# tetriscode/cause

Measured on AMD Instinct MI355X. Metric: nodes woven/sec (whole node) + % of HBM roofline at 1/2/4/8 MI355X, higher is better.
Workload: dtype u64; 1 GPU; config2: independent CausalLists, full reweave; docs_per_gpu=10000, nodes_per_doc=50001, nodes_per_gpu=500010000, sites=8, key_bits=20, key_words=u64 (cw_weave_lists), parallelism=docs sharded x1

## Files before the change

### cause_amd/csrc/causeweave.hip

```cpp

#include <hip/hip_runtime.h>

#include <algorithm>
#include <type_traits>
#include <cstdarg>
#include <cstdio>
#include <cstdlib>
#include <cstring>
#include <map>
#include <chrono>
#include <string>
#include <vector>

#include "causeweave.h"
#include "cw_internal.h"

using namespace cw;


template <int NT>
__device__ __forceinline__ uint32_t block_exscan(uint32_t v, uint32_t *wtot, uint32_t *total) {
  const int nw = NT ? NT / 64 : (int)(blockDim.x >> 6);
  const uint32_t lane = threadIdx.x & 63, w = threadIdx.x >> 6;
  uint32_t x = v;
// ... 1066 lines not shown
  }
  if (tid == 0 && bst) atomicOr(&status[d], bst);
}

constexpr uint32_t KBM_WORDS = 2 * TILE / 32;
constexpr uint32_t FRONT_FUSED_SG = 2560;

template <int NT>
__global__ __launch_bounds__(NT) void k_fplace(
    const uint32_t *__restrict__ rec_meta, const uint32_t *__restrict__ rec_par,
    const uint32_t *__restrict__ woff, const uint32_t *__restrict__ woff_base,
    const uint32_t *__restrict__ tile_start, const uint32_t *__restrict__ tile_doc,
    const uint32_t *__restrict__ tile_first, const uint32_t *__restrict__ doc_off,
    const uint64_t *__restrict__ id_key, uint32_t *__restrict__ sval, uint32_t *__restrict__ par,
    uint8_t *__restrict__ skind, uint64_t *__restrict__ skey, uint32_t *__restrict__ kbm) {
  __shared__ uint32_t s_val[TILE], s_par[TILE];
  __shared__ uint8_t s_kind[TILE];
  __shared__ uint32_t s_run[65], s_src[64];
  const uint32_t t = xcd_tile(blockIdx.x, gridDim.x), d = tile_doc[t], tid = threadIdx.x;
  const uint32_t t0 = tile_first[d], ntile = tile_first[d + 1] - t0, w = t - t0;
  const uint32_t base = doc_off[d], n = doc_off[d + 1] - base;
  const uint32_t r0 = w << 12, wlen = min(TILE, n - r0);
  if (tid < 64) {
    uint32_t a = 0, l = 0;
    if (tid < ntile) {
      const uint32_t *wo = woff + woff_base[t0 + tid];
      a = wo[w];
      l = wo[w + 1] - a;
      s_src[tid] = tile_start[t0 + tid] + a;
    }
    uint32_t x = l;
#pragma unroll
    for (int o = 1; o < 64; o <<= 1) {
      const uint32_t y = __shfl_up(x, o, 64);
      if (tid >= (uint32_t)o) x += y;
    }
    s_run[tid + 1] = x;
    if (tid == 0) s_run[0] = 0;
  }
  for (uint32_t j = tid; j < wlen; j += NT) {
    s_val[j] = 0;
    s_par[j] = 0;
    s_kind[j] = 0;
  }
  __syncthreads();
  const uint32_t total = min(s_run[ntile], wlen);
  for (uint32_t j = tid; j < total; j += NT) {
    uint32_t lo = 0, hi = ntile;
    while (hi - lo > 1) {
      const uint32_t m = (lo + hi) >> 1;
      if (s_run[m] <= j) lo = m; else hi = m;
    }
    const uint32_t g = s_src[lo] + (j - s_run[lo]);
    const uint32_t meta = rec_meta[g], rr = meta & (TILE - 1);
    s_val[rr] = (lo << 12) | ((meta >> 12) & (TILE - 1));
    s_par[rr] = rec_par[g];
    s_kind[rr] = (uint8_t)(meta >> 24);
  }
  __syncthreads();
  for (uint32_t j = tid; j < wlen; j += NT) {
    const uint32_t v = s_val[j];
    sval[base + r0 + j] = v;
    par[base + r0 + j] = s_par[j];
    skind[base + r0 + j] = s_kind[j];
    if (skey) skey[base + r0 + j] = id_key[base + (v < n ? v : 0u)];
  }
  for (uint32_t j0 = (tid >> 6) << 6; j0 < TILE; j0 += NT) {
    const uint32_t j = j0 + (tid & 63);
    const uint8_t k = j < wlen ? s_kind[j] : 0;
    const uint64_t sm = __ballot(is_special(k)), hm = __ballot(is_hide(k));
    if ((tid & 63) == 0) {
      uint32_t *o = kbm + (size_t)t * KBM_WORDS + (j0 >> 5);
      o[0] = (uint32_t)sm;
      o[1] = (uint32_t)(sm >> 32);
      o[TILE / 32] = (uint32_t)hm;
      o[TILE / 32 + 1] = (uint32_t)(hm >> 32);
    }
  }
}

__host__ __device__ inline uint32_t front_lds_bytes(uint32_t nmax, uint32_t sg) {
  return sg * 16 + 4 * ((nmax + 1) / 2) + 8 * ((nmax + 31) / 32);
}

#ifndef CW_SITE8_RANKPASS
#define CW_SITE8_RANKPASS 0
#endif
constexpr bool SITE8_PASS1 = CW_SITE8_RANKPASS == 0;

template <int NT, typename PT = uint32_t, typename VT = uint32_t, uint32_t U1 = 4, uint32_t U2 = 4,
          uint32_t U3 = 4>
__device__ __forceinline__ bool front_doc(
    const uint64_t *__restrict__ id_key, const uint64_t *__restrict__ cause_key,
    const uint8_t *__restrict__ kind, const uint32_t *__restrict__ doc_off,
    const uint32_t *__restrict__ tile_first, uint32_t sg, PT *__restrict__ par,
    uint8_t *__restrict__ skind, VT *__restrict__ sval, uint32_t *__restrict__ kbm,
    uint64_t *__restrict__ skey, uint16_t *rank16, uint64_t *__restrict__ max_ts, uint32_t ts_shift,
    uint32_t *__restrict__ status, uint32_t *__restrict__ big,
    unsigned long long *__restrict__ tprof, uint32_t d, uint4 *sdir,
    uint8_t *__restrict__ site8 = nullptr, uint32_t site_shift = 0, uint32_t site_mask = 0) {
  unsigned long long tacc[6] = {0, 0, 0, 0, 0, 0}, tlast = 0;
  auto stamp = [&](int ph) {
    if (tprof) {
      const unsigned long long now = __builtin_amdgcn_s_memtime();
      if (ph >= 0) tacc[ph] += now - tlast;
      tlast = now;
    }
  };
  stamp(-1);
  __shared__ uint64_t rmax[NT / 64];
  __shared__ uint32_t wtot[NT / 64];
  __shared__ uint32_t bst;
  const uint32_t tid = threadIdx.x, lane = tid & 63;
  const uint32_t base = doc_off[d], n = doc_off[d + 1] - base, nw = (n + 31) / 32;
  const uint64_t *const idD = id_key + base, *const causeD = cause_key + base;
  const uint8_t *const kindD = kind + base;
  uint16_t *const rankD = rank16 + base;
  PT *const parD = par + base;
  VT *const svalD = sval + base;
  uint8_t *const skindD = skind ? skind + base : nullptr;
  if (n == 0) return true;
  uint32_t *sw = reinterpret_cast<uint32_t *>(sdir);
  uint16_t *p16 = reinterpret_cast<uint16_t *>(sdir + sg);
  uint32_t *clsA = reinterpret_cast<uint32_t *>(p16) + (n + 1) / 2, *clsB = clsA + nw;
  for (uint32_t g = tid; g < sg; g += NT) sdir[g] = make_uint4(0u, 0u, 0u, 0u);
  for (uint32_t w = tid; w < nw; w += NT) clsA[w] = clsB[w] = 0;
  if (tid == 0) bst = 0;
  __syncthreads();
  const uint64_t lim = (uint64_t)sg * FR_GROUP_BITS;
  uint64_t mx = 0;
  bool dup = false, far = false;
  for (uint32_t i0 = tid; i0 < n; i0 += U1 * NT) {
    uint64_t x[U1];
#pragma unroll
    for (uint32_t u = 0; u < U1; u++) {
      const uint32_t i = i0 + u * NT;
      x[u] = i < n ? lane_at(idD, i) : 0ull;
    }
#pragma unroll
    for (uint32_t u = 0; u < U1; u++) {
      if (i0 + u * NT >= n) continue;
      mx = max(mx, x[u]);
      if (SITE8_PASS1 && site8) lane_at(site8 + base, i0 + u * NT) = (uint8_t)((x[u] >> site_shift) & site_mask);
      if (x[u] >= lim) {
        far = true;
        continue;
      }
      const uint32_t xi = (uint32_t)x[u];
      const uint32_t g = xi / FR_GROUP_BITS, b = xi - g * FR_GROUP_BITS, m = 1u << (b & 31);
      atomicOr(&sw[g * 4 + 1 + (b >> 5)], m);
    }
  }
#pragma unroll
  for (int o = 32; o > 0; o >>= 1) mx = max(mx, (uint64_t)__shfl_xor(mx, o, 64));
  if (lane == 0) rmax[tid >> 6] = mx;
  const bool any_far = __syncthreads_or(far);
  mx = rmax[0];
#pragma unroll
  for (int w = 1; w < NT / 64; w++) mx = max(mx, rmax[w]);
  if (tid == 0 && max_ts) max_ts[d] = mx >> ts_shift;
  if (any_far) {
    if (tid == 0) atomicAdd(&big[0], 1u);
    return false;
  }
  stamp(0);
  const uint32_t G = (uint32_t)(mx / FR_GROUP_BITS) + 1;
  {
    const uint32_t per = (G + NT - 1) / NT, g0 = min(G, tid * per), g1 = min(G, g0 + per);
    uint32_t cnt = 0;
    for (uint32_t g = g0; g < g1; g++) {
      const uint4 q = sdir[g];
      cnt += __popc(q.y) + __popc(q.z) + __popc(q.w);
    }
    uint32_t distinct;
    uint32_t run = block_exscan<NT>(cnt, wtot, &distinct);
    dup = distinct != n;
    for (uint32_t g = g0; g < g1; g++) {
      const uint4 q = sdir[g];
      sw[g * 4] = run;
      run += __popc(q.y) + __popc(q.z) + __popc(q.w);
    }
  }
  __syncthreads();
  const uint64_t xend = (uint64_t)G * FR_GROUP_BITS;
  uint32_t st = 0;
  uint64_t qk[U2], qc[U2];
  uint8_t qd[U2];
  auto load_group = [&](uint32_t i0) {
#pragma unroll
    for (uint32_t u = 0; u < U2; u++) {
      const uint32_t i = i0 + u * NT;
      qk[u] = i < n ? lane_at(idD, i) : 0ull;
      qc[u] = i < n ? lane_at(causeD, i) : 0ull;
      qd[u] = i < n ? lane_at(kindD, i) : 0;
    }
  };
  constexpr bool PF = U2 <= 4;
  if (PF) load_group(tid);
  for (uint32_t i0 = tid; i0 < n; i0 += U2 * NT) {
    uint64_t k[U2], c[U2];
    uint8_t kd[U2];
    if (!PF) load_group(i0);
#pragma unroll
    for (uint32_t u = 0; u < U2; u++) {
      k[u] = qk[u];
      c[u] = qc[u];
      kd[u] = qd[u];
    }
    if (PF && i0 + U2 * NT < n) load_group(i0 + U2 * NT);
#pragma unroll
    for (uint32_t u = 0; u < U2; u++) {
      const uint32_t i = i0 + u * NT;
      if (i >= n) continue;
      bool pres;
      const uint32_t r = fr_rank(sdir, (uint32_t)k[u], &pres);
      uint32_t p = 0;
      if (r == 0) {
        if (!(kd[u] & KIND_ROOT)) st |= CW_STATUS_ROOT;
      } else {
        if (kd[u] & KIND_ROOT) st |= CW_STATUS_ROOT;
        bool cp = false;
        uint32_t cr = 0;
        if (c[u] < xend) cr = fr_rank(sdir, (uint32_t)c[u], &cp);
        if (!cp) st |= CW_STATUS_ORPHAN;
        else if (c[u] >= k[u]) st |= CW_STATUS_NON_LAMPORT;
        else p = cr;
      }
      if (r < n) {
        p16[r] = (uint16_t)p;
        const uint32_t cls = kd[u] & KIND_CLASS;
        if (cls & 1) atomicOr(&clsA[r >> 5], 1u << (r & 31));
        if (cls & 2) atomicOr(&clsB[r >> 5], 1u << (r & 31));
      }
      lane_at(rankD, i) = (uint16_t)min(r, 0xFFFFu);
      if (!SITE8_PASS1 && site8) lane_at(site8 + base, i) = (uint8_t)((k[u] >> site_shift) & site_mask);
    }
  }
  if (st) atomicOr(&bst, st);
  __syncthreads();
  stamp(1);
  for (uint32_t r = tid; r < n; r += NT) {
    const uint32_t p = p16[r];
    lane_at(parD, r) = (PT)p;
    const uint32_t a = (clsA[r >> 5] >> (r & 31)) & 1u, b = (clsB[r >> 5] >> (r & 31)) & 1u;
    if (skindD) lane_at(skindD, r) = (uint8_t)(a | (b << 1));
  }
  uint32_t *kb = kbm + (size_t)tile_first[d] * KBM_WORDS;
  for (uint32_t w = tid; w < nw; w += NT) {
    const uint32_t a = clsA[w], b = clsB[w];
    uint32_t *o = kb + (size_t)(w >> 7) * KBM_WORDS + (w & 127);
    o[0] = a | b;
    o[TILE / 32] = a ^ b;
  }
  if (tid == 0 && bst) atomicOr(&status[d], bst);
  if (tid == 0 && (bst & (CW_STATUS_ROOT | CW_STATUS_ORPHAN | CW_STATUS_NON_LAMPORT)))
    atomicAdd(&big[1], 1u);
  if (__syncthreads_or(dup) && tid == 0) atomicOr(&status[d], (uint32_t)CW_STATUS_DUP);
  stamp(2);
  for (uint32_t i0 = tid; i0 < n; i0 += U3 * NT) {
    uint32_t r[U3];
#pragma unroll
    for (uint32_t u = 0; u < U3; u++) {
      const uint32_t i = i0 + u * NT;
      r[u] = i < n ? lane_at(rankD, i) : 0xFFFFu;
    }
#pragma unroll
    for (uint32_t u = 0; u < U3; u++)
      if (r[u] < n) p16[r[u]] = (uint16_t)(i0 + u * NT);
  }
  __syncthreads();
  stamp(3);
  for (uint32_t r = tid; r < n; r += NT) lane_at(svalD, r) = (VT)p16[r];
  if (skey) {
    const uint32_t per = (G + NT - 1) / NT, g0 = min(G, tid * per), g1 = min(G, g0 + per);
    for (uint32_t g = g0; g < g1; g++) {
      const uint4 q = sdir[g];
      uint32_t r = q.x;
      const uint32_t wv[3] = {q.y, q.z, q.w};
#pragma unroll
      for (uint32_t k = 0; k < 3; k++)
        for (uint32_t m = wv[k]; m != 0 && r < n; m &= m - 1)
          skey[base + r++] = (uint64_t)g * FR_GROUP_BITS + 32 * k + (uint32_t)(__ffs(m) - 1);
    }
  }
  stamp(4);
  if (tprof && tid == 0)
    for (int ph = 0; ph < 6; ph++) tprof[(size_t)d * 8 + ph] = tacc[ph];
  return true;
}

template <int NT>
__global__ __launch_bounds__(NT) void k_front(
    const uint64_t *__restrict__ id_key, const uint64_t *__restrict__ cause_key,
    const uint8_t *__restrict__ kind, const uint32_t *__restrict__ doc_off,
    const uint32_t *__restrict__ tile_first, uint32_t sg, uint32_t *__restrict__ par,
    uint8_t *__restrict__ skind, uint32_t *__restrict__ sval, uint32_t *__restrict__ kbm,
    uint64_t *__restrict__ skey, uint16_t *rank16, uint64_t *__restrict__ max_ts, uint32_t ts_shift,
    uint32_t *__restrict__ status, uint32_t *__restrict__ big,
    unsigned long long *__restrict__ tprof, uint32_t doc0 = 0) {
  extern __shared__ __attribute__((aligned(16))) uint4 lds_fr[];
  front_doc<NT>(id_key, cause_key, kind, doc_off, tile_first, sg, par, skind, sval, kbm, skey, rank16,
                max_ts, ts_shift, status, big, tprof, doc0 + blockIdx.x, lds_fr);
}

__global__ __launch_bounds__(256) void k_or_bits_at(const uint32_t *__restrict__ src, uint32_t nbits,
                                                    uint32_t *__restrict__ dst, uint32_t off) {
  const uint32_t i = blockIdx.x * blockDim.x + threadIdx.x;
  if (i * 32 >= nbits) return;
  uint32_t x = src[i];
  const uint32_t len = min(32u, nbits - i * 32);
  if (len < 32) x &= (1u << len) - 1;
  if (!x) return;
  const uint32_t p = off + i * 32, w = p >> 5, sh = p & 31;
  atomicOr(&dst[w], x << sh);
  if (sh) {
    const uint32_t hi = x >> (32 - sh);
    if (hi) atomicOr(&dst[w + 1], hi);
  }
// ... 201 lines not shown
#pragma unroll
    for (uint32_t k = 0; k < IT; k++) {
      fs4[k] = qfs[k];
      fcr[k] = qfs[k] ? qfs[k] : qfn[k];
      ns4[k] = qns[k];
    }
    if (r0 + TILE_T < n) load_tile(r0 + TILE_T);
#pragma unroll
    for (uint32_t k = 0; k < IT; k++) {
      const uint32_t j = k * NT + tid, r = r0 + j;
      flg[k] = 0;
      if (j >= len) continue;
      const bool sp = special_at(r);
      uint32_t tv;
      if (r == 0) {
        tv = RES | SUCC_END;
      } else {
        uint32_t ns = ns4[k], e = 0;
        if (ns & NSC_UP) {
          e = ns & ~NSC_UP;
          ns = sp ? dfn[k] : 0u;
        }
        if (ns) tv = RES | ns;
        else if (e >= r0) tv = e - r0;
        else if (e + TILE_T >= r0) tv = P[e + TILE_T - r0];
        else tv = RES | dth[k];
      }
      T[j] = tv;
      const uint32_t fs = fs4[k];
      const bool vis = !sp && r != 0 && !(fs && hide_at(fs));
      const bool split = r == split_node(d, r >> log2k, log2k, n);
      flg[k] = (vis ? LINK_VIS : 0u) | (split ? LINK_SPLIT : 0u);
    }
    __syncthreads();
    stamp(4);
    for (;;) {
      bool open = false;
#pragma unroll
      for (uint32_t k = 0; k < IT; k++) {
        const uint32_t j = k * NT + tid;
        if (j < len) {
          const uint32_t t0 = T[j];
          if (!(t0 & RES)) {
            const uint32_t t1 = T[t0];
            T[j] = t1;
            open |= !(t1 & RES);
          }
        }
      }
      if (!__syncthreads_or(open)) break;
    }
    stamp(5);
#pragma unroll
    for (uint32_t k = 0; k < IT; k++) {
      const uint32_t j = k * NT + tid, r = r0 + j;
      if (j >= len) continue;
      const uint32_t th = T[j] & ~RES;
      thr[base + r] = th;
      link[base + r] = (fcr[k] ? fcr[k] : th) | flg[k];
    }
    __syncthreads();
    stamp(6);
    uint32_t *x = T;
    T = P;
    P = x;
    if (r0 + TILE_T < n) load_dep(r0 + TILE_T);
  }
  if (tprof && tid == 0)
    for (int ph = 0; ph < 8; ph++) tprof[(size_t)d * 16 + ph] = tacc[ph];
}

constexpr uint32_t TL_END = 0xFFFFu;


__host__ __device__ constexpr uint32_t tree_l_tile_bytes(uint32_t nt, uint32_t tile) {
  return 4 * tile * 4 + (nt / 64) * SUB_BINS * 4 + tile * 2;
}
__host__ __device__ constexpr uint32_t tree_l_static_bytes(uint32_t nt, uint32_t tile) {
  return tree_l_tile_bytes(nt, tile) + 64 * 4 + 4;
}
__host__ __device__ inline uint32_t tree_l_lds_bytes(uint32_t nmax) {
  return ((nmax + 31) / 32) * 8 + ((nmax + 1) / 2) * 4;
}

#ifndef CW_S2_JUMP_BARRIER
#define CW_S2_JUMP_BARRIER 0
#endif
constexpr bool S2_JUMP_NOBAR = CW_S2_JUMP_BARRIER == 0;

template <int NT, int TILE_T, bool PROF, int MODE, typename PT = uint32_t>
__device__ __forceinline__ void tree_l_doc(
    const PT *__restrict__ par, const uint8_t *__restrict__ skind,
    const uint32_t *__restrict__ doc_off, const uint32_t *__restrict__ doc_log2k, uint32_t kbits,
    uint32_t bm_words, uint32_t *__restrict__ nsc, uint32_t *__restrict__ fcS,
    uint32_t *__restrict__ link, uint32_t *__restrict__ osp,
    unsigned long long *__restrict__ tprof,
    const uint32_t *__restrict__ kbm, const uint32_t *__restrict__ tile_first, uint32_t d,
    uint32_t *lds) {
  constexpr uint32_t IT = TILE_T / NT;
  unsigned long long tacc[16] = {}, tlast = 0;
  auto stamp = [&](int ph) {
    if (PROF) {
      const unsigned long long now = __builtin_amdgcn_s_memtime();
      if (ph >= 0) tacc[ph] += now - tlast;
      tlast = now;
    }
  };
  stamp(-1);
  static_assert(MODE == 4, "k_tree_l is built with direct list heads only");
  constexpr bool DH = true;
  constexpr uint32_t HS = DH ? TILE_T : 2 * TILE_T, GMAX = 16, HB = TILE_T <= 2048 ? 11 : 12;
  static_assert(TILE_T <= (1u << HB) && 17 + HB <= 32, "slot word layout");
  static_assert(2 * HS + (DH ? 2 * TILE_T : 0) == 4 * TILE_T, "hash (+ direct heads) = 4 TILE_T words");
  uint32_t *const hbuf = lds;
  uint32_t(*const wcnt)[SUB_BINS] = reinterpret_cast<uint32_t(*)[SUB_BINS]>(lds + 4 * TILE_T);
  uint16_t *const nxt = reinterpret_cast<uint16_t *>(lds + 4 * TILE_T + (NT / 64) * SUB_BINS);
  uint32_t *const bm = lds + tree_l_tile_bytes(NT, TILE_T) / 4;
  uint32_t *const hw = hbuf, *const hk = hbuf, *const hh = hbuf + HS;
  uint32_t *const tkey = hbuf, *const trank = hbuf + TILE_T, *const tns = hbuf + 2 * TILE_T;
  uint32_t *const ptab = tns;
  __shared__ uint32_t run[64];
  __shared__ uint32_t n_osp;
  const uint32_t tid = threadIdx.x;
  const uint32_t base = doc_off[d], n = doc_off[d + 1] - base, log2k = doc_log2k[d];
  const PT *const parD = par + base;
  uint32_t *const fcSD = fcS + base, *const nscD = nsc + base;
  uint32_t *const linkD = link + base, *const ospD = osp + base;
  uint32_t *const spec_bm = bm, *const hide_bm = bm + bm_words;
  uint16_t *const tab = reinterpret_cast<uint16_t *>(bm + 2 * bm_words);
  const uint32_t nw = (n + 31) >> 5;
  if (kbm) {
    const uint32_t *src = kbm + (size_t)tile_first[d] * KBM_WORDS;
    for (uint32_t wi = tid; wi < nw; wi += NT) {
      const uint32_t *tw = src + (size_t)(wi >> 7) * KBM_WORDS + (wi & 127);
      spec_bm[wi] = tw[0];
      hide_bm[wi] = tw[TILE / 32];
    }
  } else {
    for (uint32_t rb = (tid >> 6) << 6; rb < n; rb += NT) {
      const uint32_t r = rb + (tid & 63);
      const uint8_t kd = r < n ? skind[base + r] : 0;
      const uint64_t sm = __ballot(r < n && is_special(kd));
      const uint64_t hm = __ballot(r < n && is_hide(kd));
      if ((tid & 63) == 0) {
        spec_bm[rb >> 5] = (uint32_t)sm;
        hide_bm[rb >> 5] = (uint32_t)hm;
        if ((rb >> 5) + 1 < nw) {
          spec_bm[(rb >> 5) + 1] = (uint32_t)(sm >> 32);
          hide_bm[(rb >> 5) + 1] = (uint32_t)(hm >> 32);
        }
      }
    }
  }
  __syncthreads();
  stamp(0);
  auto special_at = [&](uint32_t r) -> bool { return (spec_bm[r >> 5] >> (r & 31)) & 1u; };
  auto hide_at = [&](uint32_t r) -> bool { return (hide_bm[r >> 5] >> (r & 31)) & 1u; };
  uint32_t qpar[IT];
  auto load_par = [&](uint32_t r0) {
#pragma unroll
    for (uint32_t k = 0; k < IT; k++) {
      const uint32_t r = r0 + wb_elem<IT>(k);
      qpar[k] = r < n ? lane_at(parD, r) : 0u;
    }
  };
  auto clear_hash = [&]() {
    for (uint32_t i = tid; i < HS; i += NT) {
      hw[i] = 0;
      hh[i] = TL_END;
    }
    if (DH)
// ... 170 lines not shown
          if (slot[k] < 2 * HS) hk[slot[k] - HS] = 0;
          hbuf[slot[k]] = TL_END;
        } else if (kk) {
          hw[slot[k]] = 0;
          hh[slot[k]] = TL_END;
        }
      }
      __syncthreads();
    }
    stamp(3);
  };
  uint32_t r0t = 0;
  for (; r0t + TILE_T <= n; r0t += TILE_T) tile1(r0t, std::true_type());
  if (r0t < n) tile1(r0t, std::false_type());
  for (uint32_t i = tid; i < n_osp; i += NT) {
    const uint32_t v = lane_at(ospD, i), f = tab[v & 0xFFFFu];
    if (f) lane_at(nscD, (v >> 16)) = f;
  }
  __syncthreads();
  constexpr uint32_t RES = 0x80000000u;
  uint32_t *const T = hbuf;
  struct Q {
    uint32_t fs[IT], ns[IT];
  };
  auto load_tile = [&](Q &q, uint32_t r0) {
#pragma unroll
    for (uint32_t k = 0; k < IT; k++) {
      const uint32_t r = r0 + k * NT + tid;
      const bool ok = r < n;
      q.fs[k] = ok ? lane_at(fcSD, r) : 0u;
      q.ns[k] = ok ? lane_at(nscD, r) : 0u;
    }
  };
  auto tile2f = [&](uint32_t r0, Q &X, auto fullc) {
    constexpr bool F = decltype(fullc)::value;
    const uint32_t len = F ? TILE_T : min((uint32_t)TILE_T, n - r0);
    uint32_t flg[IT], fcr[IT];
#pragma unroll
    for (uint32_t k = 0; k < IT; k++) {
      const uint32_t j = k * NT + tid, r = r0 + j;
      flg[k] = 0;
      fcr[k] = 0;
      if (j >= len) continue;
      fcr[k] = X.fs[k] ? X.fs[k] : (uint32_t)tab[r];
      const bool sp = special_at(r);
      uint32_t tv;
      if (r == 0) {
        tv = RES | SUCC_END;
      } else {
        uint32_t ns = X.ns[k], e = 0;
        if (ns & NSC_UP) {
          e = ns & ~NSC_UP;
          ns = 0;
        }
        if (ns) {
          tv = RES | ns;
        } else if (e >= r0) {
          tv = e - r0;
        } else {
          const uint32_t t = tab[e];
          tv = RES | (t == TL_END ? SUCC_END : t);
        }
      }
      T[j] = tv;
      const uint32_t fs = X.fs[k];
      const bool vis = !sp && r != 0 && !(fs && hide_at(fs));
      const bool split = r == split_node(d, r >> log2k, log2k, n);
      flg[k] = (vis ? LINK_VIS : 0u) | (split ? LINK_SPLIT : 0u);
    }
    if (r0 + 2 * TILE_T < n) load_tile(X, r0 + 2 * TILE_T);
    __syncthreads();
    stamp(5);
#pragma unroll
    for (uint32_t k = 0; k < IT; k++) {
      const uint32_t j = k * NT + tid;
      if (j < len) {
        uint32_t t = T[j];
        while (!(t & RES)) {
          t = T[t];
          T[j] = t;
        }
      }
    }
    if (!S2_JUMP_NOBAR) __syncthreads();
    stamp(6);
#pragma unroll
    for (uint32_t k = 0; k < IT; k++) {
      const uint32_t j = k * NT + tid, r = r0 + j;
      if (j >= len) continue;
      const uint32_t th = T[j] & ~RES;
      tab[r] = (uint16_t)(th == SUCC_END ? TL_END : th);
      lane_at(linkD, r) = (fcr[k] ? fcr[k] : th) | flg[k];
    }
    __syncthreads();
    stamp(7);
  };
  auto tile2 = [&](uint32_t r0, Q &X) {
    if (r0 + TILE_T <= n) tile2f(r0, X, std::true_type());
    else tile2f(r0, X, std::false_type());
  };
  Q qa, qb;
  load_tile(qa, 0);
  if (TILE_T < n) load_tile(qb, TILE_T);
  stamp(4);
  for (uint32_t r0 = 0; r0 < n; r0 += 2 * TILE_T) {
    tile2(r0, qa);
    if (r0 + TILE_T < n) tile2(r0 + TILE_T, qb);
  }
  if (PROF && tid == 0)
    for (int ph = 0; ph < 16; ph++) tprof[(size_t)d * 16 + ph] = tacc[ph];
}

template <int NT, int TILE_T, bool PROF, int MODE>
__global__ __launch_bounds__(NT) void k_tree_l(
    const uint32_t *__restrict__ par, const uint8_t *__restrict__ skind,
    const uint32_t *__restrict__ doc_off, const uint32_t *__restrict__ doc_log2k, uint32_t kbits,
    uint32_t bm_words, uint32_t *__restrict__ nsc, uint32_t *__restrict__ fcS,
    uint32_t *__restrict__ link, uint32_t *__restrict__ osp,
    unsigned long long *__restrict__ tprof,
    const uint32_t *__restrict__ kbm, const uint32_t *__restrict__ tile_first, uint32_t doc0 = 0) {
  extern __shared__ __attribute__((aligned(16))) uint32_t lds_tl[];
  tree_l_doc<NT, TILE_T, PROF, MODE>(par, skind, doc_off, doc_log2k, kbits, bm_words, nsc, fcS, link,
                                     osp, tprof, kbm, tile_first, doc0 + blockIdx.x, lds_tl);
}

constexpr uint32_t GL_TILE = 2048;
__global__ __launch_bounds__(256) void k_geff(const uint32_t *__restrict__ par,
                                              const uint8_t *__restrict__ skind, uint32_t n,
                                              uint32_t root_key, uint32_t *__restrict__ gk,
                                              uint32_t *__restrict__ fcS, uint32_t *__restrict__ fcN,
                                              uint32_t *__restrict__ zero_a,
                                              uint32_t *__restrict__ zero_b,
                                              uint32_t *__restrict__ tcnt) {
  const uint32_t r = blockIdx.x * blockDim.x + threadIdx.x;
  bool cross = false;
  if (r < n) {
    if (!tcnt) {
      fcS[r] = 0;
      fcN[r] = 0;
    }
    if (r == 0) {
      gk[0] = root_key;
      if (zero_a) *zero_a = 0;
      if (zero_b) *zero_b = 0;
    } else {
      const bool sp = is_special(skind[r]);
      uint32_t c = par[r];
      c = c < r ? c : 0u;
      if (!sp)
        while (c != 0 && is_special(skind[c])) {
          const uint32_t pc = par[c];
          c = pc < c ? pc : 0u;
        }
      gk[r] = (c << 1) | (sp ? 0u : 1u);
      cross = c < (r & ~(GL_TILE - 1));
    }
  }
  if (tcnt) {
    const uint64_t m = __ballot(cross);
    __shared__ uint32_t bc;
    if (threadIdx.x == 0) bc = 0;
    __syncthreads();
    if ((threadIdx.x & 63) == 0 && m) atomicAdd(&bc, (uint32_t)__popcll(m));
    __syncthreads();
    if (threadIdx.x == 0 && bc) atomicAdd(&tcnt[blockIdx.x * blockDim.x / GL_TILE], bc);
  }
}
// ... 593 lines not shown
    uint32_t *__restrict__ perm, uint8_t *__restrict__ vis8, uint32_t *__restrict__ vcount,
    uint32_t *__restrict__ status) {
  __shared__ uint32_t wtot[4];
  __shared__ uint32_t stage_p[EMIT_STAGE];
  __shared__ uint8_t stage_v[EMIT_STAGE];
  __shared__ uint32_t P0s;
  const uint32_t b = xcd_tile(blockIdx.x, gridDim.x), d = eblk_doc[b];
  const uint32_t base = doc_off[d], n = doc_off[d + 1] - base, f = walk_first[d];
  const uint32_t Weff = min(doc_W[d] + dyn_ctr[d], walk_first[d + 1] - f);
  const uint32_t log2cap = doc_log2cap[d], cap = 1u << log2cap;
  const uint32_t ti = eblk_x0[b] + threadIdx.x;
  uint32_t nvis = 0, cnt = 0, p0 = 0;
  bool bad = false;
  uint4 rec = make_uint4(0u, 0u, 0u, 0u);
  if (erec && ti < Weff) rec = erec[f + ti];
  const uint32_t x = ti < Weff ? (erec ? rec.x : order[f + ti]) : 0u;
  const uint4 *sl4 = nullptr;
  if (ti < Weff) {
    if (x < Weff) {
      cnt = erec ? rec.z : wcnt[f + x];
      p0 = erec ? rec.y : sbase[f + x];
      sl4 = reinterpret_cast<const uint4 *>(slots + slot_first[d] + ((size_t)x << log2cap));
      if (p0 + cnt > n || cnt > cap) bad = true;
    } else {
      bad = true;
    }
  }
  if (bad) cnt = 0;
  uint32_t total;
  const uint32_t off = block_exscan<0>(cnt, wtot, &total);
  if (threadIdx.x == 0) P0s = p0;
  __syncthreads();
  const uint32_t P0 = P0s;
  if (cnt && p0 != P0 + off) {
    bad = true;
    cnt = 0;
  }
  const bool staged = total <= EMIT_STAGE && P0 + total <= n;
  for (uint32_t k0 = 0; k0 < cnt; k0 += 4) {
    const uint4 q = sl4[k0 >> 2];
    const uint32_t e4[4] = {q.x, q.y, q.z, q.w};
#pragma unroll
    for (uint32_t u = 0; u < 4; u++) {
      const uint32_t k = k0 + u;
      if (k >= cnt) break;
      const uint32_t r = e4[u] & SLOT_IDX;
      if (r >= n) {
        bad = true;
        continue;
      }
      const uint32_t v = e4[u] >> 31;
      const uint32_t pv = sval ? sval[base + r] : r;
      if (staged) {
        stage_p[off + k] = pv;
        stage_v[off + k] = (uint8_t)v;
      } else {
        perm[base + p0 + k] = pv;
        vis8[base + p0 + k] = (uint8_t)v;
      }
      nvis += v;
    }
  }
  if (staged) {
    __syncthreads();
    for (uint32_t j = threadIdx.x; j < total; j += 256) {
      perm[base + P0 + j] = stage_p[j];
      vis8[base + P0 + j] = stage_v[j];
    }
  }
  if (bad) atomicOr(&status[d], (uint32_t)CW_STATUS_INTERNAL);
  uint32_t vtotal;
  block_exscan<0>(nvis, wtot, &vtotal);
  if (threadIdx.x == 0 && vtotal) atomicAdd(&vcount[d], vtotal);
}

constexpr uint32_t TOUR_END = 0xFFFFu;
constexpr uint32_t TOUR_LDS_MAX = 159 * 1024;

__host__ __device__ inline uint32_t tour_lds_bytes(uint32_t nmax, uint32_t log2k) {
  const uint32_t S = (nmax + (1u << log2k) - 1) >> log2k;
  return 4 * ((nmax + 1) / 2 + 2 * ((nmax + 31) / 32) + S);
}

template <int NT, typename VT = uint32_t>
__device__ __forceinline__ void tour_doc(const uint32_t *__restrict__ link,
                                             const VT *__restrict__ sval,
                                             const uint32_t *__restrict__ doc_off,
                                             const uint32_t *__restrict__ doc_log2k,
                                             const uint64_t *__restrict__ skey, uint32_t ts_shift,
                                             uint64_t *__restrict__ max_ts,
                                             uint32_t *__restrict__ perm, uint32_t *__restrict__ vbits,
                                             uint32_t *__restrict__ vcount,
                                             uint32_t *__restrict__ status, uint32_t *loc,
                                             unsigned long long *__restrict__ tprof,
                                             uint32_t d, uint32_t *sm) {
  constexpr uint32_t SPT = 8;
  __shared__ uint32_t wtot[NT / 64];
  __shared__ uint32_t bad_s, next_j;
  unsigned long long tacc[6] = {0, 0, 0, 0, 0, 0}, tlast = 0;
  auto stamp = [&](int ph) {
    if (tprof) {
      const unsigned long long now = __builtin_amdgcn_s_memtime();
      if (ph >= 0) tacc[ph] += now - tlast;
      tlast = now;
    }
  };
  stamp(-1);
  const uint32_t tid = threadIdx.x, lane = tid & 63, wv = tid >> 6;
  const uint32_t base = doc_off[d], n = doc_off[d + 1] - base, log2k = doc_log2k[d];
  const uint32_t *const linkD = link + base;
  uint32_t *const locD = loc + base, *const permD = perm + base;
  if (tid == 0 && max_ts) max_ts[d] = n ? (skey[base + n - 1] >> ts_shift) : 0ull;
  if (n == 0) return;
  const uint32_t S = (n + (1u << log2k) - 1) >> log2k, nw = (n + 31) / 32;
  uint16_t *succ = reinterpret_cast<uint16_t *>(sm);
  uint32_t *vbm = sm + (n + 1) / 2, *sbm = vbm + nw;
  uint32_t *const sub = sbm + nw;
  if (tid == 0) {
    bad_s = 0;
    next_j = NT;
  }
  constexpr uint32_t LU = 8;
  for (uint32_t r0 = wv * 64; r0 < n; r0 += NT * LU) {
    uint32_t L[LU];
#pragma unroll
    for (uint32_t k = 0; k < LU; k++) {
      const uint32_t r = r0 + k * NT + lane;
      L[k] = r < n ? lane_at(linkD, r) : 0u;
    }
#pragma unroll
    for (uint32_t k = 0; k < LU; k++) {
      const uint32_t rb = r0 + k * NT, r = rb + lane, u = L[k] & LINK_IDX;
      if (r < n) succ[r] = (uint16_t)(u < n ? u : TOUR_END);
      const uint64_t vm = __ballot(r < n && (L[k] & LINK_VIS));
      const uint64_t sp = __ballot(r < n && (L[k] & LINK_SPLIT));
      if (lane == 0 && rb < n) {
        vbm[rb >> 5] = (uint32_t)vm;
        sbm[rb >> 5] = (uint32_t)sp;
        if ((rb >> 5) + 1 < nw) {
          vbm[(rb >> 5) + 1] = (uint32_t)(vm >> 32);
          sbm[(rb >> 5) + 1] = (uint32_t)(sp >> 32);
        }
      }
    }
  }
  __syncthreads();
  stamp(0);
  bool bad = false;
  {
    uint32_t j = tid, u = 0, cnt = 0;
    bool live = j < S;
    if (live) {
      const uint32_t v = split_node(d, j, log2k, n);
      lane_at(locD, v) = j << 16;
      u = succ[v];
      cnt = 1;
    }
    while (live) {
      const uint32_t us = u < n ? u : 0u;
      const uint32_t nx = succ[us], sw = sbm[us >> 5];
      const bool end = u >= n || ((sw >> (us & 31)) & 1u) || cnt > n;
      if (end) {
        bad |= (u != TOUR_END && u >= n) || cnt > n;
        sub[j] = min(cnt, 0xFFFFu) | (u < n ? (u >> log2k) : TOUR_END) << 16;
        j = atomicAdd(&next_j, 1u);
        live = j < S;
        if (live) {
          const uint32_t v = split_node(d, j, log2k, n);
          lane_at(locD, v) = j << 16;
          u = succ[v];
          cnt = 1;
        }
      } else {
        lane_at(locD, u) = (j << 16) | cnt;
        cnt++;
        u = nx;
      }
    }
  }
  __syncthreads();
  if (tid == 0) next_j = NT;
  stamp(1);
  for (uint32_t round = 0; (1u << round) < 2 * S; round++) {
    uint32_t na[SPT], nn[SPT];
#pragma unroll
    for (uint32_t k = 0; k < SPT; k++) {
      const uint32_t j = tid + k * NT;
      if (j < S) {
        const uint32_t sj = sub[j], q = sj >> 16;
        const uint32_t sq = q < S ? sub[q] : TOUR_END << 16;
        na[k] = (sj & 0xFFFFu) + (sq & 0xFFFFu);
        nn[k] = sq >> 16;
      }
    }
    __syncthreads();
#pragma unroll
    for (uint32_t k = 0; k < SPT; k++) {
      const uint32_t j = tid + k * NT;
      if (j < S) {
        sub[j] = min(na[k], 0xFFFFu) | nn[k] << 16;
      }
    }
    __syncthreads();
  }
  stamp(2);
  if (tid == 0 && (sub[0] & 0xFFFFu) != n) bad_s = 1;
  uint16_t *out = succ;
  uint32_t *pvis = sbm;
  for (uint32_t w = tid; w < nw; w += NT) pvis[w] = 0;
  __syncthreads();
  for (uint32_t r0 = tid; r0 < n; r0 += NT * LU) {
    uint32_t lc[LU], x[LU];
#pragma unroll
    for (uint32_t k = 0; k < LU; k++) {
      const uint32_t r = r0 + k * NT;
      lc[k] = r < n ? lane_at(locD, r) : 0u;
      x[k] = r < n ? (sval ? lane_at(sval + base, r) : r) : 0u;
    }
#pragma unroll
    for (uint32_t k = 0; k < LU; k++) {
      const uint32_t r = r0 + k * NT;
      if (r >= n) continue;
      const uint32_t j = lc[k] >> 16;
      const uint32_t pos = (j < S ? n - min(sub[j] & 0xFFFFu, n) : n) + (lc[k] & 0xFFFFu);
      if (pos >= n) {
        bad = true;
        continue;
      }
      out[pos] = (uint16_t)x[k];
      if ((vbm[r >> 5] >> (r & 31)) & 1u) atomicOr(&pvis[pos >> 5], 1u << (pos & 31));
    }
  }
  __syncthreads();
  stamp(3);
  uint32_t nvis = 0;
  for (uint32_t g = tid; g < n; g += NT) lane_at(permD, g) = out[g];
  for (uint32_t w = tid; w < nw; w += NT) nvis += __popc(pvis[w]);
  if (vbits) {
    const uint32_t W0 = base >> 5, W1 = (base + n - 1) >> 5;
    for (uint32_t W = W0 + tid; W <= W1; W += NT) {
      const uint32_t lo = max(W << 5, base), hi = min((W << 5) + 32, base + n);
      const uint32_t g = lo - base, len = hi - lo, w0 = g >> 5, off = g & 31;
      uint32_t x = pvis[w0] >> off;
      if (off && w0 + 1 < nw) x |= pvis[w0 + 1] << (32 - off);
      if (len < 32) x &= (1u << len) - 1;
      x <<= lo - (W << 5);
      if (W == W0 || W == W1) {
        if (x) atomicOr(&vbits[W], x);
      } else {
        vbits[W] = x;
      }
    }
  }
  uint32_t total;
  block_exscan<NT>(nvis, wtot, &total);
  if (__syncthreads_or(bad) || bad_s) {
    if (tid == 0) atomicOr(&status[d], (uint32_t)CW_STATUS_INTERNAL);
  }
  if (tid == 0) vcount[d] = total;
  stamp(4);
  if (tprof && tid == 0)
    for (int ph = 0; ph < 6; ph++) tprof[(size_t)d * 8 + ph] = tacc[ph];
}

template <int NT>
__global__ __launch_bounds__(NT) void k_tour(const uint32_t *__restrict__ link,
                                             const uint32_t *__restrict__ sval,
                                             const uint32_t *__restrict__ doc_off,
                                             const uint32_t *__restrict__ doc_log2k,
                                             const uint64_t *__restrict__ skey, uint32_t ts_shift,
                                             uint64_t *__restrict__ max_ts,
                                             uint32_t *__restrict__ perm, uint32_t *__restrict__ vbits,
                                             uint32_t *__restrict__ vcount,
                                             uint32_t *__restrict__ status, uint32_t *loc,
                                             unsigned long long *__restrict__ tprof,
                                             uint32_t doc0 = 0) {
  extern __shared__ __attribute__((aligned(16))) uint32_t lds_t[];
  tour_doc<NT>(link, sval, doc_off, doc_log2k, skey, ts_shift, max_ts, perm, vbits, vcount, status, loc, tprof, doc0 + blockIdx.x, lds_t);
}

template <int NT, int TILE_T, typename VT, bool PROF, int TLM = 0, int FV = 0>
__global__ __launch_bounds__(NT) void k_weave_doc(
    const uint64_t *__restrict__ id_key, const uint64_t *__restrict__ cause_key,
    const uint8_t *__restrict__ kind, const uint32_t *__restrict__ doc_off,
    const uint32_t *__restrict__ tile_first, uint32_t sg, uint16_t *__restrict__ par,
    uint8_t *__restrict__ skind, VT *__restrict__ sval, uint32_t *__restrict__ kbm,
    uint64_t *__restrict__ skey, uint16_t *rank16, uint64_t *__restrict__ max_ts, uint32_t ts_shift,
    uint32_t *__restrict__ status, uint32_t *__restrict__ big, const uint32_t *__restrict__ doc_log2k,
    uint32_t kbits, uint32_t bm_words, uint32_t *__restrict__ nsc, uint32_t *__restrict__ fcS,
    uint32_t *__restrict__ link, uint32_t *__restrict__ osp, uint32_t *__restrict__ perm,
    uint32_t *__restrict__ vbits, uint32_t *__restrict__ vcount, uint32_t *loc,
    unsigned long long *__restrict__ tprof, uint8_t *__restrict__ site8, uint32_t site_shift,
    uint32_t site_mask) {
  extern __shared__ __attribute__((aligned(16))) uint32_t lds_w[];
  const uint32_t d = blockIdx.x;
  const unsigned long long t0 = PROF ? __builtin_amdgcn_s_memtime() : 0ull;
  constexpr uint32_t U1 = FV == 0 ? 4 : 16, U2 = 6, U3 = U1;
  if (!front_doc<NT, uint16_t, VT, U1, U2, U3>(id_key, cause_key, kind, doc_off, tile_first, sg, par, skind, sval, kbm, skey,
                     rank16, max_ts, ts_shift, status, big, nullptr, d,
                     reinterpret_cast<uint4 *>(lds_w), site8, site_shift, site_mask))
    return;
  __syncthreads();
  const unsigned long long t1 = PROF ? __builtin_amdgcn_s_memtime() : 0ull;
  tree_l_doc<NT, TILE_T, false, TLM, uint16_t>(par, skind, doc_off, doc_log2k, kbits, bm_words, nsc, fcS, link,
                                   osp, nullptr, kbm, tile_first, d, lds_w);
  __syncthreads();
  const unsigned long long t2 = PROF ? __builtin_amdgcn_s_memtime() : 0ull;
  tour_doc<NT, VT>(link, sval, doc_off, doc_log2k, nullptr, 0u, nullptr, perm, vbits, vcount, status,
                   loc, nullptr, d, lds_w);
  if (PROF && threadIdx.x == 0) {
    const unsigned long long t3 = __builtin_amdgcn_s_memtime();
    tprof[(size_t)d * 4] = t1 - t0;
    tprof[(size_t)d * 4 + 1] = t2 - t1;
    tprof[(size_t)d * 4 + 2] = t3 - t2;
  }
}

__host__ __device__ inline uint32_t yarn_lds_bytes(uint32_t nmax) {
  return (nmax + 3) & ~3u;
}

template <int NT>
__global__ __launch_bounds__(NT) void k_yarn_doc(const uint8_t *__restrict__ site8,
                                                 const uint16_t *__restrict__ rank16,
                                                 const uint16_t *__restrict__ sval16,
                                                 const uint32_t *__restrict__ doc_off,
                                                 uint32_t *__restrict__ yarn) {
  extern __shared__ __attribute__((aligned(16))) uint32_t lds_y[];
  __shared__ uint32_t wrow[NT / 64][16];
  const uint32_t tid = threadIdx.x;
  const uint32_t d = blockIdx.x;
  const uint32_t base = doc_off[d], n = doc_off[d + 1] - base;
  uint8_t *const sr = reinterpret_cast<uint8_t *>(lds_y);
  for (uint32_t w = tid; w < (n + 3) / 4; w += NT) lds_y[w] = 0xFFFFFFFFu;
  constexpr uint32_t NW = NT / 64;
  const uint32_t perw = ((n + NW - 1) / NW + 63) & ~63u;
  for (uint32_t w = tid; w < NW * 16; w += NT) (&wrow[0][0])[w] = 0;
  __syncthreads();
  constexpr uint32_t U = 16;
  for (uint32_t i0 = tid; i0 < n; i0 += U * NT) {
    uint32_t x[U], r[U];
#pragma unroll
    for (uint32_t u = 0; u < U; u++) {
      const uint32_t i = i0 + u * NT;
      x[u] = i < n ? lane_at(site8 + base, i) : 0u;
      r[u] = i < n ? lane_at(rank16 + base, i) : 0xFFFFu;
    }
#pragma unroll
    for (uint32_t u = 0; u < U; u++)
      if (r[u] < n) {
        sr[r[u]] = (uint8_t)x[u];
        atomicAdd(&wrow[r[u] / perw][x[u] & 15u], 1u);
      }
  }
  __syncthreads();
  {
    const uint32_t lane = tid & 63, wv = tid >> 6;
    const uint32_t w0 = min(n, wv * perw), w1 = min(n, w0 + perw);
    auto site_mask = [&](uint32_t st, uint64_t valid, uint64_t b0, uint64_t b1, uint64_t b2,
                         uint64_t b3) -> uint64_t {
      return valid & ((st & 1u) ? b0 : ~b0) & ((st & 2u) ? b1 : ~b1) & ((st & 4u) ? b2 : ~b2) &
             ((st & 8u) ? b3 : ~b3);
    };
    uint32_t before = 0, tot = 0;
    if (lane < 16) {
#pragma unroll 1
      for (uint32_t i = 0; i < NW; i++) {
        const uint32_t t = wrow[i][lane];
        before += i < wv ? t : 0u;
        tot += t;
      }
    }
    uint32_t ex = tot;
#pragma unroll
    for (uint32_t o = 1; o < 16; o <<= 1) {
      const uint32_t y = __shfl_up(ex, o, 64);
      if (lane >= o) ex += y;
    }
    uint32_t off = ex - tot + before;
    const uint16_t *const svD = sval16 + base;
    uint32_t *const yD = yarn + base;
    constexpr uint32_t PB = 8;
    for (uint32_t c0 = w0; c0 < w1; c0 += PB * 64) {
      uint32_t v[PB];
#pragma unroll
      for (uint32_t k = 0; k < PB; k++) {
        const uint32_t r = c0 + k * 64 + lane;
        v[k] = r < w1 ? svD[r] : 0u;
      }
#pragma unroll
      for (uint32_t k = 0; k < PB; k++) {
// ... 3380 lines not shown
```

Measured before the change: 40.51 billion nodes/s.

## Overlap tour link loads with prior stage and replace sublist doubling with async chase

The fused kernel now drops the barrier between tree_l_doc and tour_doc and issues the first link loads before a barrier inside tour_doc. The link-to-successor/bitmap pass is software-pipelined with double-buffered register queues and full-tile fast paths. The barrier-separated pointer-doubling over sublists becomes a barrier-free per-thread chase using relaxed LDS atomics, capped at S trips. The placement loop also gets a full-tile specialisation, and dead compile-time flags are removed. The barrier-free chase relies on relaxed atomic visibility in LDS and could run up to S sequential trips when sublist chains are long.

```diff
diff --git a/cause_amd/csrc/causeweave.hip b/cause_amd/csrc/causeweave.hip
--- a/cause_amd/csrc/causeweave.hip
+++ b/cause_amd/csrc/causeweave.hip
@@ -1172,11 +1172,6 @@
 __host__ __device__ inline uint32_t front_lds_bytes(uint32_t nmax, uint32_t sg) {
   return sg * 16 + 4 * ((nmax + 1) / 2) + 8 * ((nmax + 31) / 32);
 }
-
-#ifndef CW_SITE8_RANKPASS
-#define CW_SITE8_RANKPASS 0
-#endif
-constexpr bool SITE8_PASS1 = CW_SITE8_RANKPASS == 0;
 
 template <int NT, typename PT = uint32_t, typename VT = uint32_t, uint32_t U1 = 4, uint32_t U2 = 4,
           uint32_t U3 = 4>
@@ -1231,7 +1226,7 @@
     for (uint32_t u = 0; u < U1; u++) {
       if (i0 + u * NT >= n) continue;
       mx = max(mx, x[u]);
-      if (SITE8_PASS1 && site8) lane_at(site8 + base, i0 + u * NT) = (uint8_t)((x[u] >> site_shift) & site_mask);
+      if (site8) lane_at(site8 + base, i0 + u * NT) = (uint8_t)((x[u] >> site_shift) & site_mask);
       if (x[u] >= lim) {
         far = true;
         continue;
@@ -1323,7 +1318,6 @@
         if (cls & 2) atomicOr(&clsB[r >> 5], 1u << (r & 31));
       }
       lane_at(rankD, i) = (uint16_t)min(r, 0xFFFFu);
-      if (!SITE8_PASS1 && site8) lane_at(site8 + base, i) = (uint8_t)((k[u] >> site_shift) & site_mask);
     }
   }
   if (st) atomicOr(&bst, st);
@@ -1691,11 +1685,6 @@
 __host__ __device__ inline uint32_t tree_l_lds_bytes(uint32_t nmax) {
   return ((nmax + 31) / 32) * 8 + ((nmax + 1) / 2) * 4;
 }
-
-#ifndef CW_S2_JUMP_BARRIER
-#define CW_S2_JUMP_BARRIER 0
-#endif
-constexpr bool S2_JUMP_NOBAR = CW_S2_JUMP_BARRIER == 0;
 
 template <int NT, int TILE_T, bool PROF, int MODE, typename PT = uint32_t>
 __device__ __forceinline__ void tree_l_doc(
@@ -2032,7 +2021,6 @@
         }
       }
     }
-    if (!S2_JUMP_NOBAR) __syncthreads();
     stamp(6);
 #pragma unroll
     for (uint32_t k = 0; k < IT; k++) {
@@ -2792,7 +2780,7 @@
   return 4 * ((nmax + 1) / 2 + 2 * ((nmax + 31) / 32) + S);
 }
 
-template <int NT, typename VT = uint32_t>
+template <int NT, typename VT = uint32_t, bool SYNC_IN = false>
 __device__ __forceinline__ void tour_doc(const uint32_t *__restrict__ link,
                                              const VT *__restrict__ sval,
                                              const uint32_t *__restrict__ doc_off,
@@ -2826,32 +2814,57 @@
   uint16_t *succ = reinterpret_cast<uint16_t *>(sm);
   uint32_t *vbm = sm + (n + 1) / 2, *sbm = vbm + nw;
   uint32_t *const sub = sbm + nw;
+  constexpr uint32_t LU = 8, LG = NT * LU;
+  struct LQ {
+    uint32_t v[LU];
+  };
+  auto load_g = [&](LQ &q, uint32_t g0) {
+    if (g0 + LG <= n) {
+#pragma unroll
+      for (uint32_t k = 0; k < LU; k++) q.v[k] = lane_at(linkD, g0 + k * NT + tid);
+    } else {
+#pragma unroll
+      for (uint32_t k = 0; k < LU; k++) {
+        const uint32_t r = g0 + k * NT + tid;
+        q.v[k] = r < n ? lane_at(linkD, r) : 0u;
+      }
+    }
+  };
+  auto take_gf = [&](const LQ &q, uint32_t g0, auto fullc) {
+    constexpr bool F = decltype(fullc)::value;
+#pragma unroll
+    for (uint32_t k = 0; k < LU; k++) {
+      const uint32_t rb = g0 + k * NT + wv * 64, r = rb + lane, u = q.v[k] & LINK_IDX;
+      if (F || r < n) succ[r] = (uint16_t)(u < n ? u : TOUR_END);
+      const uint64_t vm = __ballot((F || r < n) && (q.v[k] & LINK_VIS));
+      const uint64_t sp = __ballot((F || r < n) && (q.v[k] & LINK_SPLIT));
+      if (lane == 0 && (F || rb < n)) {
+        vbm[rb >> 5] = (uint32_t)vm;
+        sbm[rb >> 5] = (uint32_t)sp;
+        if (F || (rb >> 5) + 1 < nw) {
+          vbm[(rb >> 5) + 1] = (uint32_t)(vm >> 32);
+          sbm[(rb >> 5) + 1] = (uint32_t)(sp >> 32);
+        }
+      }
+    }
+  };
+  auto take_g = [&](const LQ &q, uint32_t g0) {
+    if (g0 + LG <= n) take_gf(q, g0, std::true_type());
+    else take_gf(q, g0, std::false_type());
+  };
+  LQ qa, qb;
+  load_g(qa, 0);
+  if (SYNC_IN) __syncthreads();
   if (tid == 0) {
     bad_s = 0;
     next_j = NT;
   }
-  constexpr uint32_t LU = 8;
-  for (uint32_t r0 = wv * 64; r0 < n; r0 += NT * LU) {
-    uint32_t L[LU];
-#pragma unroll
-    for (uint32_t k = 0; k < LU; k++) {
-      const uint32_t r = r0 + k * NT + lane;
-      L[k] = r < n ? lane_at(linkD, r) : 0u;
-    }
-#pragma unroll
-    for (uint32_t k = 0; k < LU; k++) {
-      const uint32_t rb = r0 + k * NT, r = rb + lane, u = L[k] & LINK_IDX;
-      if (r < n) succ[r] = (uint16_t)(u < n ? u : TOUR_END);
-      const uint64_t vm = __ballot(r < n && (L[k] & LINK_VIS));
-      const uint64_t sp = __ballot(r < n && (L[k] & LINK_SPLIT));
-      if (lane == 0 && rb < n) {
-        vbm[rb >> 5] = (uint32_t)vm;
-        sbm[rb >> 5] = (uint32_t)sp;
-        if ((rb >> 5) + 1 < nw) {
-          vbm[(rb >> 5) + 1] = (uint32_t)(vm >> 32);
-          sbm[(rb >> 5) + 1] = (uint32_t)(sp >> 32);
-        }
-      }
+  for (uint32_t g0 = 0; g0 < n; g0 += 2 * LG) {
+    if (g0 + LG < n) load_g(qb, g0 + LG);
+    take_g(qa, g0);
+    if (g0 + LG < n) {
+      if (g0 + 2 * LG < n) load_g(qa, g0 + 2 * LG);
+      take_g(qb, g0 + LG);
     }
   }
   __syncthreads();
@@ -2891,46 +2904,53 @@
   __syncthreads();
   if (tid == 0) next_j = NT;
   stamp(1);
-  for (uint32_t round = 0; (1u << round) < 2 * S; round++) {
-    uint32_t na[SPT], nn[SPT];
+  {
+    uint32_t w[SPT];
+    bool open = false;
 #pragma unroll
     for (uint32_t k = 0; k < SPT; k++) {
       const uint32_t j = tid + k * NT;
-      if (j < S) {
-        const uint32_t sj = sub[j], q = sj >> 16;
-        const uint32_t sq = q < S ? sub[q] : TOUR_END << 16;
-        na[k] = (sj & 0xFFFFu) + (sq & 0xFFFFu);
-        nn[k] = sq >> 16;
-      }
-    }
-    __syncthreads();
-#pragma unroll
-    for (uint32_t k = 0; k < SPT; k++) {
-      const uint32_t j = tid + k * NT;
-      if (j < S) {
-        sub[j] = min(na[k], 0xFFFFu) | nn[k] << 16;
-      }
-    }
-    __syncthreads();
-  }
-  stamp(2);
-  if (tid == 0 && (sub[0] & 0xFFFFu) != n) bad_s = 1;
+      w[k] = j < S ? sub[j] : TOUR_END << 16;
+      open |= (w[k] >> 16) < S;
+    }
+    for (uint32_t trip = 0; open && trip < S; trip++) {
+      uint32_t sq[SPT];
+#pragma unroll
+      for (uint32_t k = 0; k < SPT; k++) {
+        const uint32_t q = w[k] >> 16;
+        sq[k] = __atomic_load_n(&sub[q < S ? q : 0u], __ATOMIC_RELAXED);
+      }
+      open = false;
+#pragma unroll
+      for (uint32_t k = 0; k < SPT; k++) {
+        if ((w[k] >> 16) < S) {
+          w[k] = min((w[k] & 0xFFFFu) + (sq[k] & 0xFFFFu), 0xFFFFu) | (sq[k] & 0xFFFF0000u);
+          __atomic_store_n(&sub[tid + k * NT], w[k], __ATOMIC_RELAXED);
+          open |= (w[k] >> 16) < S;
+        }
+      }
+    }
+    bad |= open;
+  }
   uint16_t *out = succ;
   uint32_t *pvis = sbm;
   for (uint32_t w = tid; w < nw; w += NT) pvis[w] = 0;
   __syncthreads();
-  for (uint32_t r0 = tid; r0 < n; r0 += NT * LU) {
+  stamp(2);
+  if (tid == 0 && (sub[0] & 0xFFFFu) != n) bad_s = 1;
+  auto place_gf = [&](uint32_t g0, auto fullc) {
+    constexpr bool F = decltype(fullc)::value;
     uint32_t lc[LU], x[LU];
 #pragma unroll
     for (uint32_t k = 0; k < LU; k++) {
-      const uint32_t r = r0 + k * NT;
-      lc[k] = r < n ? lane_at(locD, r) : 0u;
-      x[k] = r < n ? (sval ? lane_at(sval + base, r) : r) : 0u;
+      const uint32_t r = g0 + k * NT + tid;
+      lc[k] = F || r < n ? lane_at(locD, r) : 0u;
+      x[k] = F || r < n ? (sval ? lane_at(sval + base, r) : r) : 0u;
     }
 #pragma unroll
     for (uint32_t k = 0; k < LU; k++) {
-      const uint32_t r = r0 + k * NT;
-      if (r >= n) continue;
+      const uint32_t r = g0 + k * NT + tid;
+      if (!F && r >= n) continue;
       const uint32_t j = lc[k] >> 16;
       const uint32_t pos = (j < S ? n - min(sub[j] & 0xFFFFu, n) : n) + (lc[k] & 0xFFFFu);
       if (pos >= n) {
@@ -2940,7 +2960,10 @@
       out[pos] = (uint16_t)x[k];
       if ((vbm[r >> 5] >> (r & 31)) & 1u) atomicOr(&pvis[pos >> 5], 1u << (pos & 31));
     }
-  }
+  };
+  uint32_t gt = 0;
+  for (; gt + LG <= n; gt += LG) place_gf(gt, std::true_type());
+  if (gt < n) place_gf(gt, std::false_type());
   __syncthreads();
   stamp(3);
   uint32_t nvis = 0;
@@ -3014,9 +3037,8 @@
   const unsigned long long t1 = PROF ? __builtin_amdgcn_s_memtime() : 0ull;
   tree_l_doc<NT, TILE_T, false, TLM, uint16_t>(par, skind, doc_off, doc_log2k, kbits, bm_words, nsc, fcS, link,
                                    osp, nullptr, kbm, tile_first, d, lds_w);
-  __syncthreads();
   const unsigned long long t2 = PROF ? __builtin_amdgcn_s_memtime() : 0ull;
-  tour_doc<NT, VT>(link, sval, doc_off, doc_log2k, nullptr, 0u, nullptr, perm, vbits, vcount, status,
+  tour_doc<NT, VT, true>(link, sval, doc_off, doc_log2k, nullptr, 0u, nullptr, perm, vbits, vcount, status,
                    loc, nullptr, d, lds_w);
   if (PROF && threadIdx.x == 0) {
     const unsigned long long t3 = __builtin_amdgcn_s_memtime();
```

New measurement: 40.30 billion nodes/s. Within noise of the previous version (-0.5%).
